# ushariRanasinghe/G2VLM

Hardware: AMD Instinct MI355X
Metric: views/sec (multi-view recon, G2VLM-2B-MoT) (higher is better)
Workload: dtype bf16; 1 GPU; C3: 8-view 518x518 reconstruction, full depth (24 DINO + 28 MoT + 15 decoder blocks), 1 scene per GPU; Lq=10968, Lk=10976, parallelism=replicas x1

## Files before the change

### g2vlm_amd/csrc/attn.hip

```cpp
#include <type_traits>
#include <utility>
#include "common.h"
#include "lds_dma.h"
#include "g2vlm_hip.h"

namespace {

#ifdef EXP_NO_EXP
#define G2V_EXP2(x) (x)
#else
#define G2V_EXP2(x) __builtin_amdgcn_exp2f(x)
#endif

constexpr int KV_TILE = 64;
constexpr int ROWB = 256;
constexpr int TILE_B = KV_TILE * ROWB;

struct FlashArgs {
  const __bf16* q; const __bf16* k; const __bf16* v; __bf16* o;
  const g2v_attn_tile* tiles;
  const g2v_attn_seg* segs;
  const int* seg_ptr;
  const int* comb;
  float* ws;
  int ldq, ldk, ldv, ldo, n_tiles, Hq, Hkv, n_blocks;
  float scale_log2;
#ifdef EXP_STAMPS
  unsigned long long* dbg;
  unsigned long long* clk;
  int dbg_pos;
#endif
};

#ifdef EXP_STAMPS
constexpr int STAMP_TILES = 24, STAMP_PTS = 8;
unsigned long long* g_attn_dbg = nullptr;
int g_attn_dbg_pos = -1;
unsigned long long* g_attn_clk = nullptr;
#define G2V_CLK_BEGIN() const unsigned long long clk_c0 = __builtin_amdgcn_s_memtime(), clk_r0 = __builtin_amdgcn_s_memrealtime()
#define G2V_CLK_END(lbv, wv) do { if (a.clk && (wv) == 0 && (threadIdx.x & 63) == 0) { a.clk[2 * (lbv)] = __builtin_amdgcn_s_memtime() - clk_c0; \
    a.clk[2 * (lbv) + 1] = __builtin_amdgcn_s_memrealtime() - clk_r0; } } while (0)
// ... 521 lines not shown
          const int kr = min(kt * KV_TILE + piece_row(i), T.k_len - 1);
          dma16_vaddr(base + ((size_t)kr * a.ldk + piece_col(i)) * 2, __builtin_amdgcn_readfirstlane(lds_addr(dst)) + piece_dst(i));
        }
      }
    };

    stage_any(kbase, smK, kt0);
    stage_any(vbase, smV, kt0);
    if (kt0 + 1 < kt1) { stage_any(kbase, smK, kt0 + 1); stage_any(vbase, smV, kt0 + 1); }
    if (kt0 + 2 < kt1) stage_any(kbase, smK, kt0 + 2);

    {
      auto q_to_acc = [&](auto qb_t) {
        constexpr int qb = decltype(qb_t)::value;
        const int qi = min(64 * wu + 32 * qb + r, T.q_rows - 1);
        const __bf16* qp = a.q + (size_t)(T.q0 + qi) * a.ldq + head * D + 8 * hh;
        u32x4 qv[KSTEPS];
#pragma unroll
        for (int ks = 0; ks < KSTEPS; ++ks) qv[ks] = *reinterpret_cast<const u32x4*>(qp + 16 * ks);
        auto put = [&](auto ks_t) {
          constexpr int ks = decltype(ks_t)::value, R = ACC_Q + 4 * (8 * qb + ks);
          acc_write<R>(qv[ks][0]); acc_write<R + 1>(qv[ks][1]); acc_write<R + 2>(qv[ks][2]); acc_write<R + 3>(qv[ks][3]);
        };
        put(std::integral_constant<int, 0>{}); put(std::integral_constant<int, 1>{}); put(std::integral_constant<int, 2>{});
        put(std::integral_constant<int, 3>{}); put(std::integral_constant<int, 4>{}); put(std::integral_constant<int, 5>{});
        put(std::integral_constant<int, 6>{}); put(std::integral_constant<int, 7>{});
      };
      q_to_acc(std::integral_constant<int, 0>{});
      q_to_acc(std::integral_constant<int, 1>{});
      acc_zero_seq<ACC_O>(std::make_integer_sequence<int, 128>{});
      acc_zero_seq<ACC_L>(std::make_integer_sequence<int, 32>{});
      wait32();
    }
    const int kmax0 = (T.q0 - T.q_win0) + 64 * wu + r + T.causal_shift;
// ... 332 lines not shown
          const float wgt = __builtin_amdgcn_exp2f(mv[u] - M);
          L = fmaf(lv[u], wgt, L);
#pragma unroll
          for (int e = 0; e < 4; ++e) acc[e] = fmaf(ov[u][e], wgt, acc[e]);
        }
      }
    }
    const float inv = 1.0f / L;
    __bf16* op = a.o + (size_t)(T.q0 + q) * a.ldo + head * D + 4 * c;
    *reinterpret_cast<u32x2*>(op) = u32x2{pack_bf16x2(acc[0] * inv, acc[1] * inv), pack_bf16x2(acc[2] * inv, acc[3] * inv)};
  }
}

int g_attn_form = 1;

template <int D>
int launch_flash(const FlashArgs& a, int n_comb, int waves, hipStream_t s) {
  if (a.n_blocks > 0) {
    if (D == 128 && waves == 8 && g_attn_form == 1 && a.ldk == a.ldv) hipLaunchKernelGGL(flash_fwd64_kernel, dim3(a.n_blocks), dim3(256), 0, s, a);
    else if (waves == 8) hipLaunchKernelGGL((flash_fwd_kernel<D, 8>), dim3(a.n_blocks), dim3(512), 0, s, a);
    else hipLaunchKernelGGL((flash_fwd_kernel<D, 4>), dim3(a.n_blocks), dim3(256), 0, s, a);
    G2V_CHECK_LAUNCH();
  }
  if (n_comb > 0) {
    hipLaunchKernelGGL(flash_combine_kernel<D>, dim3(n_comb, (32 * waves + COMB_ROWS - 1) / COMB_ROWS), dim3(256), 0, s, a);
    G2V_CHECK_LAUNCH();
  }
  return G2V_OK;
}

}

#ifdef EXP_STAMPS
extern "C" int g2v_debug_attn_stamps(void* buf) { g_attn_dbg = (unsigned long long*)buf; return 0; }
extern "C" int g2v_debug_attn_stamp_pos(int pos) { g_attn_dbg_pos = pos; return 0; }
extern "C" int g2v_debug_attn_clock(void* buf) { g_attn_clk = (unsigned long long*)buf; return 0; }
#endif

extern "C" int g2v_debug_attn_form(int form) { g_attn_form = form; return 0; }

extern "C" int64_t g2v_flash_attn_workspace(int n_slots) { return (int64_t)(n_slots > 0 ? n_slots : 0) * SLOT_FLOATS * 4; }

extern "C" int g2v_flash_attn(const void* q, int ldq, const void* k, int ldk, const void* v, int ldv, void* o, int ldo,
                              const g2v_attn_tile* tiles, int n_tiles, int Hq, int Hkv, int D, float scale,
                              const g2v_attn_seg* segs, const int32_t* seg_ptr, int n_blocks, const int32_t* comb, int n_comb,
                              int tile_rows, void* workspace, void* stream) {
  if (!q || !k || !v || !o || !tiles || n_tiles < 0 || Hq <= 0 || Hkv <= 0 || Hq % Hkv || n_blocks < 0 || n_comb < 0) return G2V_ERR_ARG;
  if ((n_blocks > 0 && (!segs || !seg_ptr)) || (n_comb > 0 && (!comb || !workspace))) return G2V_ERR_ARG;
  if ((ldq & 7) || (ldk & 7) || (ldv & 7) || (ldo & 3)) return G2V_ERR_ARG;
  if (tile_rows != 128 && tile_rows != 256) return G2V_ERR_ARG;
  if (n_tiles == 0 || (n_blocks == 0 && n_comb == 0)) return G2V_OK;
  FlashArgs a{(const __bf16*)q, (const __bf16*)k, (const __bf16*)v, (__bf16*)o, tiles, segs, seg_ptr, comb,
              (float*)workspace, ldq, ldk, ldv, ldo, n_tiles, Hq, Hkv, n_blocks, scale * 1.4426950408889634f};
#ifdef EXP_STAMPS
  a.dbg = g_attn_dbg;
  a.dbg_pos = g_attn_dbg_pos;
  a.clk = g_attn_clk;
#endif
  const int waves = tile_rows / 32;
  hipStream_t s = (hipStream_t)stream;
  switch (D) {
    case 16: return launch_flash<16>(a, n_comb, waves, s);
    case 64: return launch_flash<64>(a, n_comb, waves, s);
    case 80: return launch_flash<80>(a, n_comb, waves, s);
    case 96: return launch_flash<96>(a, n_comb, waves, s);
    case 128: return launch_flash<128>(a, n_comb, waves, s);
    default: return G2V_ERR_ARG;
  }
}
```

### g2vlm_amd/csrc/common.h

```cpp
#pragma once
#include <hip/hip_runtime.h>
#include <stdint.h>

typedef __attribute__((ext_vector_type(8))) __bf16 bf16x8;
typedef __attribute__((ext_vector_type(4))) __bf16 bf16x4;
typedef __attribute__((ext_vector_type(2))) __bf16 bf16x2;
typedef __attribute__((ext_vector_type(4))) short s16x4;
typedef __attribute__((ext_vector_type(4))) float f32x4;
typedef __attribute__((ext_vector_type(16))) float f32x16;
typedef __attribute__((ext_vector_type(4))) uint32_t u32x4;
typedef __attribute__((ext_vector_type(2))) uint32_t u32x2;

#define G2V_OK 0
#define G2V_ERR_ARG (-22)
#define G2V_ERR_LAUNCH (-5)

#define G2V_CHECK_LAUNCH()                         \
  do {                                             \
    hipError_t e__ = hipGetLastError();            \
    if (e__ != hipSuccess) return G2V_ERR_LAUNCH;  \
  } while (0)

__device__ __forceinline__ float bf2f(__bf16 x) { return (float)x; }
__device__ __forceinline__ __bf16 f2bf(float x) { return (__bf16)x; }
__device__ __forceinline__ float bfround(float x) {
  uint32_t r;
  asm("v_cvt_pk_bf16_f32 %0, %1, %1" : "=v"(r) : "v"(x));
  return __uint_as_float(r << 16);
}

__device__ __forceinline__ float bits2f_hi(uint32_t w) { return __uint_as_float(w & 0xffff0000u); }
__device__ __forceinline__ float bits2f_lo(uint32_t w) { return __uint_as_float(w << 16); }

__device__ __forceinline__ uint32_t pack_bf16x2(float lo, float hi) {
  bf16x2 v = {(__bf16)lo, (__bf16)hi};
  return *reinterpret_cast<uint32_t*>(&v);
}

__device__ __forceinline__ float wave_sum(float v) {
#pragma unroll
  for (int o = 32; o > 0; o >>= 1) v += __shfl_xor(v, o, 64);
  return v;
}
__device__ __forceinline__ float wave_max(float v) {
#pragma unroll
  for (int o = 32; o > 0; o >>= 1) v = fmaxf(v, __shfl_xor(v, o, 64));
  return v;
}

__device__ __forceinline__ float gelu_erf(float x) { return 0.5f * x * (1.0f + erff(x * 0.70710678118654752440f)); }
__device__ __forceinline__ float gelu_fast(float x) {
  const float a = fabsf(x) * 0.70710678118654752440f;
  const float t = __builtin_amdgcn_rcpf(fmaf(0.5f, a, 1.0f));
// ... 19 lines not shown
```

### g2vlm_amd/csrc/norm_rope.hip

```cpp
#include "common.h"
#include "g2vlm_hip.h"

namespace {


template <bool IN_BF16, int MAXV>
__device__ __forceinline__ int load_row(const void* x, size_t row_off, int C, int lane, f32x4 (&v)[MAXV]) {
  int n = 0;
#pragma unroll
  for (int i = 0; i < MAXV; ++i) {
    int c = (i * 64 + lane) * 4;
    v[i] = f32x4{0.f, 0.f, 0.f, 0.f};
    if (c < C) {
      if constexpr (IN_BF16) {
        u32x2 w = *reinterpret_cast<const u32x2*>(reinterpret_cast<const __bf16*>(x) + row_off + c);
        v[i] = f32x4{bits2f_lo(w[0]), bits2f_hi(w[0]), bits2f_lo(w[1]), bits2f_hi(w[1])};
      } else {
        v[i] = *reinterpret_cast<const f32x4*>(reinterpret_cast<const float*>(x) + row_off + c);
      }
      n = i + 1;
    }
  }
  return n;
}
// ... 89 lines not shown
  const int nh = Hq + 2 * Hkv;
  const long item = ((long)blockIdx.x * 256 + threadIdx.x) >> 4;
  const bool live = item < (long)L * nh;
  const long it = live ? item : 0;
  const int row = (int)(it / nh), h = (int)(it - (long)row * nh);
  const int j = threadIdx.x & 15;
  const __bf16* src = qkv + (size_t)row * nh * 128 + h * 128 + 4 * j;
  u32x2 a = *reinterpret_cast<const u32x2*>(src), b = *reinterpret_cast<const u32x2*>(src + 64);
  if (h >= Hq + Hkv) {
    if (live) {
      __bf16* dst = v_cache + ((size_t)kv_rows[row] * Hkv + (h - Hq - Hkv)) * 128 + 4 * j;
      *reinterpret_cast<u32x2*>(dst) = a; *reinterpret_cast<u32x2*>(dst + 64) = b;
    }
    return;
  }
  float x0[4] = {bits2f_lo(a[0]), bits2f_hi(a[0]), bits2f_lo(a[1]), bits2f_hi(a[1])};
  float x1[4] = {bits2f_lo(b[0]), bits2f_hi(b[0]), bits2f_lo(b[1]), bits2f_hi(b[1])};
  float ss = 0.f;
#pragma unroll
  for (int e = 0; e < 4; ++e) ss += x0[e] * x0[e] + x1[e] * x1[e];
#pragma unroll
  for (int o = 8; o > 0; o >>= 1) ss += __shfl_xor(ss, o, 64);
  const float rstd = 1.0f / sqrtf(ss / 128.f + eps);
  const bool isq = h < Hq;
  const float* w = (isq ? (row < split ? qw_lo : qw_hi) : (row < split ? kw_lo : kw_hi)) + 4 * j;
  const f32x4 w0 = *reinterpret_cast<const f32x4*>(w), w1 = *reinterpret_cast<const f32x4*>(w + 64);
  const float* cp = cs + (size_t)row * 128 + 4 * j; const float* sp = sn + (size_t)row * 128 + 4 * j;
  const f32x4 c0 = *reinterpret_cast<const f32x4*>(cp), c1 = *reinterpret_cast<const f32x4*>(cp + 64);
  const f32x4 s0 = *reinterpret_cast<const f32x4*>(sp), s1 = *reinterpret_cast<const f32x4*>(sp + 64);
  float o0[4], o1[4];
#pragma unroll
  for (int e = 0; e < 4; ++e) {
    float n0 = __fmul_rn(x0[e], rstd), n1 = __fmul_rn(x1[e], rstd);
    if (und_rounding) { n0 = bfround(n0); n1 = bfround(n1); }
    n0 = __fmul_rn(w0[e], n0); n1 = __fmul_rn(w1[e], n1);
    o0[e] = __fadd_rn(__fmul_rn(n0, c0[e]), __fmul_rn(-n1, s0[e]));
    o1[e] = __fadd_rn(__fmul_rn(n1, c1[e]), __fmul_rn(n0, s1[e]));
  }
  if (live) {
    __bf16* dst = (isq ? q_out + ((size_t)row * Hq + h) * 128 : k_cache + ((size_t)kv_rows[row] * Hkv + (h - Hq)) * 128) + 4 * j;
    *reinterpret_cast<u32x2*>(dst) = u32x2{pack_bf16x2(o0[0], o0[1]), pack_bf16x2(o0[2], o0[3])};
    *reinterpret_cast<u32x2*>(dst + 64) = u32x2{pack_bf16x2(o1[0], o1[1]), pack_bf16x2(o1[2], o1[3])};
  }
}

__global__ void rope2d_kernel(__bf16* x, int ld, int M, int col0, int n_heads, int D, const __bf16* cs, const __bf16* sn,
                              const int* pos, int P) {
  const int half = D / 2, quarter = D / 4;
  int per_row = n_heads * half;
  long i = (long)blockIdx.x * blockDim.x + threadIdx.x;
  if (i >= (long)M * per_row) return;
  int row = (int)(i / per_row), r = (int)(i - (long)row * per_row);
  int h = r / half, e = r - h * half;
  int axis = e / quarter, j = e - axis * quarter;
  int p = pos[(row % P) * 2 + axis];
  __bf16* t = x + (size_t)row * ld + col0 + h * D + axis * half;
  float t0 = bf2f(t[j]), t1 = bf2f(t[j + quarter]);
// ... 97 lines not shown
                                      const void* kw_lo, const void* kw_hi, int split, float eps, int und_rounding,
                                      const void* cos, const void* sin, void* q_out, void* k_cache, void* v_cache,
                                      const void* kv_rows, void* stream) {
  if (!qkv || !qw_lo || !qw_hi || !kw_lo || !kw_hi || !cos || !sin || !q_out || !k_cache || !v_cache || !kv_rows ||
      L < 0 || Hq <= 0 || Hkv <= 0) return G2V_ERR_ARG;
  if (L == 0) return G2V_OK;
  long items = (long)L * (Hq + 2 * Hkv);
  hipLaunchKernelGGL(qknorm_mrope_cache_kernel, dim3((unsigned)((items + 15) / 16)), dim3(256), 0, (hipStream_t)stream,
                     (const __bf16*)qkv, L, Hq, Hkv, (const float*)qw_lo, (const float*)qw_hi, (const float*)kw_lo,
                     (const float*)kw_hi, split, eps, und_rounding, (const float*)cos, (const float*)sin, (__bf16*)q_out,
                     (__bf16*)k_cache, (__bf16*)v_cache, (const int*)kv_rows);
  G2V_CHECK_LAUNCH();
  return G2V_OK;
}

extern "C" int g2v_rope2d(void* x, int ld, int M, int col0, int n_heads, int D, const void* cos, const void* sin,
                          const void* pos, int P, void* stream) {
  if (!x || !cos || !sin || !pos || M < 0 || n_heads <= 0 || D <= 0 || (D & 3) || P <= 0) return G2V_ERR_ARG;
  if (M == 0) return G2V_OK;
  long n = (long)M * n_heads * (D / 2);
  if ((D & 15) == 0 && (ld & 3) == 0 && (col0 & 3) == 0 && (reinterpret_cast<uintptr_t>(x) & 7) == 0 &&
      ((reinterpret_cast<uintptr_t>(cos) | reinterpret_cast<uintptr_t>(sin)) & 7) == 0) {
    n /= 4;
    hipLaunchKernelGGL(rope2d_vec4_kernel, dim3((unsigned)((n + 255) / 256)), dim3(256), 0, (hipStream_t)stream, (__bf16*)x, ld, M,
                       col0, n_heads, D, (const __bf16*)cos, (const __bf16*)sin, (const int*)pos, P);
    G2V_CHECK_LAUNCH();
    return G2V_OK;
  }
  hipLaunchKernelGGL(rope2d_kernel, dim3((unsigned)((n + 255) / 256)), dim3(256), 0, (hipStream_t)stream, (__bf16*)x, ld, M, col0,
                     n_heads, D, (const __bf16*)cos, (const __bf16*)sin, (const int*)pos, P);
// ... 14 lines not shown
```

### g2vlm_amd/engine.py

```python
import math
import os

import torch

from . import hip
from .decode import Decode, KVCache, linear_names, weight_key


def rope2d_tables(D, seq_len, base=100.0):
    inv_freq = 1.0 / (base ** (torch.arange(0, D, 2).float() / D))
    t = torch.arange(seq_len, dtype=inv_freq.dtype)
    freqs = torch.einsum("i,j->ij", t, inv_freq).to(torch.bfloat16)
    freqs = torch.cat((freqs, freqs), dim=-1)
    return freqs.cos(), freqs.sin()


def attn_tile_rows(windows, Hq):
    long_kv = sum(w[3] for w in windows if w[0] == windows[0][0]) >= 2048 and max(w[1] for w in windows) >= 2048
    tall = False
    if not long_kv:
        pad = lambda t: sum((w[1] + t - 1) // t * t for w in windows) / max(1, sum(w[1] for w in windows))
        items = sum((w[1] + 255) // 256 for w in windows) * Hq
        tall = items >= 512 and pad(256) <= 1.12 * pad(128)
    return 256 if (long_kv or tall) else 128
# ... 119 lines not shown
            assert not causal and local_kv is not None
            r0, nr = local_kv
            wins = [(0, L, r0, nr, False, 0)]
            if r0 > 0:
                wins.append((0, L, 0, r0, False, 1))
            if r0 + nr < tot:
                wins.append((0, L, r0 + nr, tot - r0 - nr, False, 1))
            plan = self.plan(tuple(wins), Hq)
        elif windows is not None:
            plan = self.plan(tuple(windows), Hq)
        else:
            plan = self.plan(((0, L, 0, tot, bool(causal)),), Hq)
        nq, nqkv = Hq * 128, (Hq + 2 * Hkv) * 128
        h = torch.empty((L, H), dtype=torch.bfloat16, device=self.dev)
        qkv = torch.empty((L, nqkv), dtype=torch.bfloat16, device=self.dev)
        qb = torch.empty((L, nq), dtype=torch.bfloat16, device=self.dev)
        ao = torch.empty((L, nq), dtype=torch.bfloat16, device=self.dev)
        act = torch.empty((L, Lc["ffn"]), dtype=torch.bfloat16, device=self.dev)
        ng, nu = split, L - split

        def groups(A, C, wname, bname=None, res=None, gamma=None, lda=None, ldc=None):
            gs = []
            for tag, r0, m, gam in (("geo", 0, ng, gamma), ("und", split, nu, None)):
                if m == 0:
                    continue
                gs.append(dict(A=A[r0:], W=w[wname.format(tag)], bias=w[bname.format(tag)] if bname else None,
                               C=C[r0:], res=res[r0:] if res is not None else None, gamma=gam, M=m))
            return gs

        for i in range(Lc["layers"] if num_layers is None else num_layers):
            p = f"L{i}."
            hp.rmsnorm(x, w[p + "geo.ln1"], w[p + "und.ln1"], split, eps, out=h)
            hp.gemm_bf16(groups(h, qkv, p + "{}.qkv.w", p + "{}.qkv.b"), nqkv, H, hp.EPI_BF16, out_ld=nqkv)
            hp.qknorm_mrope_cache(qkv, Hq, Hkv, w[p + "geo.qn"], w[p + "und.qn"], w[p + "geo.kn"], w[p + "und.kn"], split, eps,
                                  und_rounding, cos, sin, qb, cache.k[i], cache.v[i], kv_rows)
            if self.attn_events is not None:
                ev = (torch.cuda.Event(enable_timing=True), torch.cuda.Event(enable_timing=True))
                ev[0].record()
            kk, vv_ = cache.k[i][:tot].view(tot, Hkv * 128), cache.v[i][:tot].view(tot, Hkv * 128)
            if kv_exchange is not None:
                kv_exchange.start(i)
                hp.flash_attn(qb, kk, vv_, ao, plan, Hq, Hkv, 128, phase=0)
                kv_exchange.wait(i)
                for ph in range(1, len(plan.phases)):
                    hp.flash_attn(qb, kk, vv_, ao, plan, Hq, Hkv, 128, phase=ph)
            else:
                hp.flash_attn(qb, kk, vv_, ao, plan, Hq, Hkv, 128)
            if self.attn_events is not None:
                ev[1].record()
                self.attn_events.append((ev, L, tot))
            hp.gemm_bf16(groups(ao, x, p + "{}.o.w", None, res=x, gamma=w[p + "ls1"]), H, nq, hp.EPI_RES_F32, out_ld=H, ldres=H,
                         flags=hp.GAMMA_ROUND_BF16)
            hp.rmsnorm(x, w[p + "geo.ln2"], w[p + "und.ln2"], split, eps, out=h)
            if self.gemm_events is not None:
                gev = (torch.cuda.Event(enable_timing=True), torch.cuda.Event(enable_timing=True))
                gev[0].record()
            hp.gemm_bf16(groups(h, act, p + "{}.gu.w"), 2 * Lc["ffn"], H, hp.EPI_SWIGLU, out_ld=Lc["ffn"])
            if self.gemm_events is not None:
                gev[1].record()
                self.gemm_events.append((gev, L))
            hp.gemm_bf16(groups(act, x, p + "{}.down.w", None, res=x, gamma=w[p + "ls2"]), H, Lc["ffn"], hp.EPI_RES_F32, out_ld=H,
                         ldres=H, lda=Lc["ffn"], flags=hp.GAMMA_ROUND_BF16)
# ... 189 lines not shown
```

### g2vlm_amd/hip.py

```python
import ctypes as C
import os
import threading

import torch

_HERE = os.path.dirname(os.path.abspath(__file__))
LIB_PATH = os.environ.get("G2V_LIB_PATH") or os.path.join(_HERE, "lib", "libg2vlm_hip.so")

EPI_BF16, EPI_GELU, EPI_QUICKGELU, EPI_SWIGLU, EPI_RES_F32, EPI_RES_BF16 = range(6)
GAMMA_ROUND_BF16 = 1
FORCE_SMALL_TILE = 2
SUPERTILE = 4
FORCE_BIG_TILE = 8
FORCE_8P = 16
P8_H192, P8_H128, P8_H256, P8_TWO_BARRIER, P8_H288, P8_H224, P8_H160 = 128, 256, 512, 1024, 4096, 8192, 16384
P8_PIPELINED = 32768
P8_FOUR_WAVES = 65536
P8_EIGHT_WAVES = 131072
P8_NO_ROW_SKIP = 262144
F32, BF16 = 0, 1
NO_CAUSAL = 2 ** 30
_DEBUG_GEMM_FLAGS = int(os.environ.get("G2V_GEMM_FLAGS", "0"))


# ... 8 lines not shown
                ("flags", C.c_int32), ("workspace", C.c_void_p), ("workspace_bytes", C.c_int64)]


_P, _I, _F, _L = C.c_void_p, C.c_int, C.c_float, C.c_int64
_SIGS = {
    "g2v_version": ([], C.c_int),
    "g2v_arch": ([], C.c_char_p),
    "g2v_gemm_bf16": ([C.POINTER(GemmDesc), _P], C.c_int),
    "g2v_gemm_route": ([C.POINTER(GemmDesc), C.POINTER(C.c_int32 * 4)], C.c_int),
    "g2v_gemm_f32": ([_P, _P, _P, _P, _P, _I, _I, _I, _I, _I, _I, _I, _P], C.c_int),
    "g2v_layernorm": ([_P, _I, _I, _P, _P, _F, _P, _I, _I, _I, _I, _P], C.c_int),
    "g2v_rmsnorm": ([_P, _I, _P, _P, _I, _F, _P, _I, _I, _I, _I, _P], C.c_int),
    "g2v_mrope_table": ([_P, _I, _P, _P, _P, _P], C.c_int),
    "g2v_qknorm_mrope_cache": ([_P, _I, _I, _I, _P, _P, _P, _P, _I, _F, _I, _P, _P, _P, _P, _P, _P, _P], C.c_int),
    "g2v_flash_attn": ([_P, _I, _P, _I, _P, _I, _P, _I, _P, _I, _I, _I, _I, _F, _P, _P, _I, _P, _I, _I, _P, _P], C.c_int),
    "g2v_flash_attn_workspace": ([_I], C.c_int64),
    "g2v_debug_attn_form": ([_I], C.c_int),
    "g2v_rope2d": ([_P, _I, _I, _I, _I, _I, _P, _P, _P, _I, _P], C.c_int),
    "g2v_rope_vision": ([_P, _I, _I, _I, _I, _P, _P, _P], C.c_int),
    "g2v_im2col14": ([_P, _I, _I, _I, _P, _I, _P], C.c_int),
    "g2v_dino_preprocess": ([_P, _I, _I, _I, _I, C.POINTER(C.c_float), C.POINTER(C.c_float), _P, _P, _P], C.c_int),
    "g2v_dino_assemble": ([_P, _P, _P, _P, _P, _I, _I, _I, _P], C.c_int),
    "g2v_im2col_patch": ([_P, _I, _I, _I, _I, _P, _I, _P], C.c_int),
    "g2v_qwen_patchify_u8": ([_P, _I, _I, _I, C.POINTER(C.c_float), C.POINTER(C.c_float), _P, _I, _P], C.c_int),
    "g2v_vit_assemble": ([_P, _P, _P, _P, _I, _I, _I, _I, _P], C.c_int),
    "g2v_gather_rows_f32": ([_P, _I, _P, _P, _I, _I, _I, _P], C.c_int),
    "g2v_scatter_rows_f32": ([_P, _I, _P, _P, _I, _I, _I, _P], C.c_int),
    "g2v_cast_f32_bf16": ([_P, _P, _L, _P], C.c_int),
    "g2v_cast_bf16_f32": ([_P, _P, _L, _P], C.c_int),
    "g2v_pts_epilogue": ([_P, _I, _I, _I, _I, _P, _P, _P, _P], C.c_int),
# ... 194 lines not shown

def mrope_table(pos_i32, inv_freq):
    L = pos_i32.shape[1]
    cos = torch.empty((L, 128), dtype=torch.float32, device=pos_i32.device)
    sin = torch.empty_like(cos)
    _ck(lib().g2v_mrope_table(_p(pos_i32), L, _p(inv_freq), _p(cos), _p(sin), _stream()), "g2v_mrope_table")
    return cos, sin


def qknorm_mrope_cache(qkv, Hq, Hkv, qw_lo, qw_hi, kw_lo, kw_hi, split, eps, und_rounding, cos, sin, q_out, k_cache,
                       v_cache, kv_rows):
    L = qkv.shape[0]
    _ck(lib().g2v_qknorm_mrope_cache(_p(qkv), L, Hq, Hkv, _p(qw_lo), _p(qw_hi), _p(kw_lo), _p(kw_hi), int(split), eps,
                                     int(und_rounding), _p(cos), _p(sin), _p(q_out), _p(k_cache), _p(v_cache),
                                     _p(kv_rows), _stream()), "g2v_qknorm_mrope_cache")


class AttnSeg(C.Structure):
    _fields_ = [("desc", C.c_int32), ("head", C.c_int32), ("kt0", C.c_int32), ("kt1", C.c_int32), ("slot", C.c_int32),
                ("_pad", C.c_int32 * 3)]


class AttnPlan:

    def __init__(self, tiles, n_tiles, phases, comb, n_comb, n_slots, tile_rows, device):
        self.tiles, self.n_tiles, self.phases = tiles, n_tiles, phases
        self.comb, self.n_comb, self.n_slots, self.tile_rows = comb, n_comb, n_slots, tile_rows
        self.n_blocks = max((p[2] for p in phases), default=0)
        self.n_split = n_comb
        self.ws_words = max(4, int(lib().g2v_flash_attn_workspace(n_slots)) // 4)
# ... 103 lines not shown
        ptr, k = [0], 0
        for lst in per_block:
            for (i, kt0, kt1) in lst:
                d, h = items[i][0], items[i][1]
                sg = segs[k]
                sg.desc, sg.head, sg.kt0, sg.kt1, sg.slot = d, h, kt0, kt1, slot_of[(d, h, kt0)]
                k += 1
            ptr.append(k)
        seg_t = torch.frombuffer(bytearray(bytes(segs)), dtype=torch.int32).clone()
        phases.append((h2d(seg_t, device, resident=True), h2d(torch.tensor(ptr, dtype=torch.int32), device, resident=True), n_blocks))
    tiles = h2d(torch.tensor(rows, dtype=torch.int32).reshape(-1, 8), device, resident=True)
    comb_t = h2d(torch.tensor(comb if comb else [0, 0, 0, 0], dtype=torch.int32), device, resident=True)
    return AttnPlan(tiles, n_tiles, phases, comb_t, len(comb) // 4, n_slots, tile_rows, device)


def flash_attn(q, k, v, out, plan, Hq, Hkv, D, scale=None, phase=None):
    scale = scale if scale is not None else D ** -0.5
    ws = plan.ws(scratch_owner(q.device.index))
    last = len(plan.phases) - 1
    for i in (range(len(plan.phases)) if phase is None else (phase,)):
        segs, seg_ptr, n_blocks = plan.phases[i]
        n_comb = plan.n_comb if i == last else 0
        _ck(lib().g2v_flash_attn(_p(q), _rowmajor(q), _p(k), _rowmajor(k), _p(v), _rowmajor(v), _p(out), _rowmajor(out),
                                 _p(plan.tiles), plan.n_tiles, Hq, Hkv, D, scale, _p(segs), _p(seg_ptr), n_blocks, _p(plan.comb), n_comb,
                                 plan.tile_rows, _p(ws), _stream()), "g2v_flash_attn")
    return out


def rope2d(x, col0, n_heads, D, cos, sin, pos, P):
    _ck(lib().g2v_rope2d(_p(x), _rowmajor(x), x.shape[0], col0, n_heads, D, _p(cos), _p(sin), _p(pos), P, _stream()),
        "g2v_rope2d")


def rope_vision(x, n_heads, D, cos, sin):
    _ck(lib().g2v_rope_vision(_p(x), _rowmajor(x), x.shape[0], n_heads, D, _p(cos), _p(sin), _stream()), "g2v_rope_vision")


# ... 333 lines not shown
```

### include/g2vlm_hip.h

```cpp
#ifndef G2VLM_HIP_H
#define G2VLM_HIP_H
#include <stdint.h>
#ifdef __cplusplus
extern "C" {
#endif

int g2v_version(void);
const char* g2v_arch(void);

enum {
  G2V_EPI_BF16 = 0,
  G2V_EPI_GELU = 1,
  G2V_EPI_QUICKGELU = 2,
  G2V_EPI_SWIGLU = 3,
  G2V_EPI_RES_F32 = 4,
  G2V_EPI_RES_BF16 = 5
};
#define G2V_GEMM_GAMMA_ROUND_BF16 1
#define G2V_GEMM_SUPERTILE 4
#define G2V_GEMM_FORCE_BIG_TILE 8
#define G2V_GEMM_FORCE_8P 16
#define G2V_GEMM_8P_H192 128
#define G2V_GEMM_8P_H128 256
#define G2V_GEMM_8P_H256 512
// ... 32 lines not shown
                 int M, int N, int K, int lda, int ldc, int ldres, int relu, void* stream);

#define G2V_F32 0
#define G2V_BF16 1
int g2v_layernorm(const void* x, int x_dtype, int ldx, const void* w, const void* b, float eps,
                  void* out, int out_dtype, int ldo, int M, int C, void* stream);
int g2v_rmsnorm(const void* x, int ldx, const void* w_lo, const void* w_hi, int split, float eps,
                void* out, int out_dtype, int ldo, int M, int C, void* stream);

int g2v_mrope_table(const void* pos, int L, const void* inv_freq , void* cos, void* sin, void* stream);
int g2v_qknorm_mrope_cache(const void* qkv, int L, int Hq, int Hkv,
                           const void* qw_lo, const void* qw_hi, const void* kw_lo, const void* kw_hi,
                           int split, float eps, int und_rounding, const void* cos, const void* sin,
                           void* q_out, void* k_cache, void* v_cache, const void* kv_rows, void* stream);

typedef struct {
  int32_t q0, q_rows;
  int32_t k0, k_len;
  int32_t causal_shift;
  int32_t q_win0;
  int32_t _pad[2];
} g2v_attn_tile;

typedef struct {
  int32_t desc;
  int32_t head;
  int32_t kt0, kt1;
  int32_t slot;
  int32_t _pad[3];
} g2v_attn_seg;
int64_t g2v_flash_attn_workspace(int n_slots);
int g2v_debug_attn_form(int form);
int g2v_flash_attn(const void* q, int ldq, const void* k, int ldk, const void* v, int ldv,
                   void* o, int ldo, const g2v_attn_tile* tiles, int n_tiles,
                   int Hq, int Hkv, int D, float scale,
                   const g2v_attn_seg* segs, const int32_t* seg_ptr, int n_blocks, const int32_t* comb, int n_comb,
                   int tile_rows, void* workspace, void* stream);

int g2v_rope2d(void* x, int ld, int M, int col0, int n_heads, int D, const void* cos, const void* sin,
               const void* pos, int P, void* stream);

int g2v_rope_vision(void* x, int ld, int M, int n_heads, int D, const void* cos, const void* sin, void* stream);

int g2v_dino_preprocess(const void* in, int in_is_u8, int N, int H, int W, const float* mean3, const float* std3, void* norm,
                        void* orig, void* stream);

int g2v_lanczos_resize_u8(const void* src, int N, int Hin, int Win, void* dst, int Hout, int Wout, void* tmp,
                          const void* bounds_h, const void* kk_h, int ksize_h,
                          const void* bounds_v, const void* kk_v, int ksize_v, void* stream);
int g2v_im2col14(const void* img, int N, int H, int W, void* out, int Kpad, void* stream);
int g2v_dino_assemble(const void* patch, const void* cls, const void* regs, const void* pos,
                      void* x, int N, int P, int C, void* stream);

// ... 88 lines not shown
```

Before: 105.1 views/s.

## Fuse Q RMSNorm and mRoPE into flash attention Q load

Q-head RMSNorm and mRoPE move out of the separate qknorm_mrope_cache kernel and into the fwd64 attention kernel's Q-load prologue. Attention reads raw Q straight from the qkv buffer. A new K-only norm/rope kernel still fills the KV cache and copies V. This drops the round trip of the normalized Q buffer through memory and removes its allocation. In exchange every attention block recomputes the norm and rope for its Q rows, repeated per KV segment or phase, which adds register pressure to the hot kernel. The rounding also changes from explicit _rn ops to fmaf.

```diff
diff --git a/g2vlm_amd/csrc/attn.hip b/g2vlm_amd/csrc/attn.hip
--- a/g2vlm_amd/csrc/attn.hip
+++ b/g2vlm_amd/csrc/attn.hip
@@ -25,6 +25,9 @@
   float* ws;
   int ldq, ldk, ldv, ldo, n_tiles, Hq, Hkv, n_blocks;
   float scale_log2;
+  const float* qw_lo; const float* qw_hi; const float* cs; const float* sn;
+  int split, und_rounding;
+  float eps;
 #ifdef EXP_STAMPS
   unsigned long long* dbg;
   unsigned long long* clk;
@@ -576,10 +579,41 @@
       auto q_to_acc = [&](auto qb_t) {
         constexpr int qb = decltype(qb_t)::value;
         const int qi = min(64 * wu + 32 * qb + r, T.q_rows - 1);
-        const __bf16* qp = a.q + (size_t)(T.q0 + qi) * a.ldq + head * D + 8 * hh;
+        const int qrow = T.q0 + qi;
+        const __bf16* qp = a.q + (size_t)qrow * a.ldq + head * D + 8 * hh;
         u32x4 qv[KSTEPS];
 #pragma unroll
         for (int ks = 0; ks < KSTEPS; ++ks) qv[ks] = *reinterpret_cast<const u32x4*>(qp + 16 * ks);
+        if (a.cs != nullptr) {
+          float wsum[2];
+#pragma unroll
+          for (int b = 0; b < 2; ++b) {
+            float sq[4];
+#pragma unroll
+            for (int ks = 0; ks < 4; ++ks)
+              sq[ks] = qk_quad_sumsq(u32x2{qv[ks][2 * b], qv[ks][2 * b + 1]}, u32x2{qv[ks + 4][2 * b], qv[ks + 4][2 * b + 1]});
+            const float v4 = (sq[0] + sq[2]) + (sq[1] + sq[3]);
+            auto sw = __builtin_amdgcn_permlane32_swap(__float_as_uint(v4), __float_as_uint(v4), false, false);
+            wsum[b] = __uint_as_float(sw[0]) + __uint_as_float(sw[1]);
+          }
+          const float rstd = qk_rstd128(wsum[0] + wsum[1], a.eps);
+          const float* wp = (qrow < a.split ? a.qw_lo : a.qw_hi) + 8 * hh;
+          const float* cp = a.cs + (size_t)qrow * 128 + 8 * hh;
+          const float* sp = a.sn + (size_t)qrow * 128 + 8 * hh;
+#pragma unroll
+          for (int ks = 0; ks < 4; ++ks) {
+#pragma unroll
+            for (int b = 0; b < 2; ++b) {
+              const int d = 16 * ks + 4 * b;
+              const f32x4 w0 = *reinterpret_cast<const f32x4*>(wp + d), w1 = *reinterpret_cast<const f32x4*>(wp + 64 + d);
+              const f32x4 cc = *reinterpret_cast<const f32x4*>(cp + d), ss = *reinterpret_cast<const f32x4*>(sp + d);
+              u32x2 xa = {qv[ks][2 * b], qv[ks][2 * b + 1]}, xb = {qv[ks + 4][2 * b], qv[ks + 4][2 * b + 1]};
+              qk_quad_norm_rope(xa, xb, rstd, a.und_rounding, w0, w1, cc, cc, ss, ss);
+              qv[ks][2 * b] = xa[0]; qv[ks][2 * b + 1] = xa[1];
+              qv[ks + 4][2 * b] = xb[0]; qv[ks + 4][2 * b + 1] = xb[1];
+            }
+          }
+        }
         auto put = [&](auto ks_t) {
           constexpr int ks = decltype(ks_t)::value, R = ACC_Q + 4 * (8 * qb + ks);
           acc_write<R>(qv[ks][0]); acc_write<R + 1>(qv[ks][1]); acc_write<R + 2>(qv[ks][2]); acc_write<R + 3>(qv[ks][3]);
@@ -942,10 +976,12 @@
 
 int g_attn_form = 1;
 
+bool takes_fwd64(int D, int waves, int ldk, int ldv) { return D == 128 && waves == 8 && g_attn_form == 1 && ldk == ldv; }
+
 template <int D>
 int launch_flash(const FlashArgs& a, int n_comb, int waves, hipStream_t s) {
   if (a.n_blocks > 0) {
-    if (D == 128 && waves == 8 && g_attn_form == 1 && a.ldk == a.ldv) hipLaunchKernelGGL(flash_fwd64_kernel, dim3(a.n_blocks), dim3(256), 0, s, a);
+    if (takes_fwd64(D, waves, a.ldk, a.ldv)) hipLaunchKernelGGL(flash_fwd64_kernel, dim3(a.n_blocks), dim3(256), 0, s, a);
     else if (waves == 8) hipLaunchKernelGGL((flash_fwd_kernel<D, 8>), dim3(a.n_blocks), dim3(512), 0, s, a);
     else hipLaunchKernelGGL((flash_fwd_kernel<D, 4>), dim3(a.n_blocks), dim3(256), 0, s, a);
     G2V_CHECK_LAUNCH();
@@ -969,17 +1005,24 @@
 
 extern "C" int64_t g2v_flash_attn_workspace(int n_slots) { return (int64_t)(n_slots > 0 ? n_slots : 0) * SLOT_FLOATS * 4; }
 
-extern "C" int g2v_flash_attn(const void* q, int ldq, const void* k, int ldk, const void* v, int ldv, void* o, int ldo,
-                              const g2v_attn_tile* tiles, int n_tiles, int Hq, int Hkv, int D, float scale,
-                              const g2v_attn_seg* segs, const int32_t* seg_ptr, int n_blocks, const int32_t* comb, int n_comb,
-                              int tile_rows, void* workspace, void* stream) {
+namespace {
+int flash_attn_impl(const void* q, int ldq, const void* k, int ldk, const void* v, int ldv, void* o, int ldo,
+                    const g2v_attn_tile* tiles, int n_tiles, int Hq, int Hkv, int D, float scale, const g2v_attn_seg* segs,
+                    const int32_t* seg_ptr, int n_blocks, const int32_t* comb, int n_comb, int tile_rows, void* workspace,
+                    const g2v_attn_qprep* qp, void* stream) {
   if (!q || !k || !v || !o || !tiles || n_tiles < 0 || Hq <= 0 || Hkv <= 0 || Hq % Hkv || n_blocks < 0 || n_comb < 0) return G2V_ERR_ARG;
   if ((n_blocks > 0 && (!segs || !seg_ptr)) || (n_comb > 0 && (!comb || !workspace))) return G2V_ERR_ARG;
   if ((ldq & 7) || (ldk & 7) || (ldv & 7) || (ldo & 3)) return G2V_ERR_ARG;
   if (tile_rows != 128 && tile_rows != 256) return G2V_ERR_ARG;
+  if (qp && (!qp->qw_lo || !qp->qw_hi || !qp->cos || !qp->sin || !takes_fwd64(D, tile_rows / 32, ldk, ldv))) return G2V_ERR_ARG;
   if (n_tiles == 0 || (n_blocks == 0 && n_comb == 0)) return G2V_OK;
   FlashArgs a{(const __bf16*)q, (const __bf16*)k, (const __bf16*)v, (__bf16*)o, tiles, segs, seg_ptr, comb,
-              (float*)workspace, ldq, ldk, ldv, ldo, n_tiles, Hq, Hkv, n_blocks, scale * 1.4426950408889634f};
+              (float*)workspace, ldq, ldk, ldv, ldo, n_tiles, Hq, Hkv, n_blocks, scale * 1.4426950408889634f,
+              nullptr, nullptr, nullptr, nullptr, 0, 0, 0.f};
+  if (qp) {
+    a.qw_lo = (const float*)qp->qw_lo; a.qw_hi = (const float*)qp->qw_hi; a.cs = (const float*)qp->cos; a.sn = (const float*)qp->sin;
+    a.split = qp->split; a.und_rounding = qp->und_rounding; a.eps = qp->eps;
+  }
 #ifdef EXP_STAMPS
   a.dbg = g_attn_dbg;
   a.dbg_pos = g_attn_dbg_pos;
@@ -996,3 +1039,25 @@
     default: return G2V_ERR_ARG;
   }
 }
+}
+
+extern "C" int g2v_flash_attn(const void* q, int ldq, const void* k, int ldk, const void* v, int ldv, void* o, int ldo,
+                              const g2v_attn_tile* tiles, int n_tiles, int Hq, int Hkv, int D, float scale,
+                              const g2v_attn_seg* segs, const int32_t* seg_ptr, int n_blocks, const int32_t* comb, int n_comb,
+                              int tile_rows, void* workspace, void* stream) {
+  return flash_attn_impl(q, ldq, k, ldk, v, ldv, o, ldo, tiles, n_tiles, Hq, Hkv, D, scale, segs, seg_ptr, n_blocks, comb, n_comb,
+                         tile_rows, workspace, nullptr, stream);
+}
+
+extern "C" int g2v_flash_attn_qprep_supported(int D, int tile_rows, int ldk, int ldv) {
+  return (tile_rows == 128 || tile_rows == 256) && takes_fwd64(D, tile_rows / 32, ldk, ldv) ? 1 : 0;
+}
+
+extern "C" int g2v_flash_attn_qprep(const void* qkv, int ldq, const void* k, int ldk, const void* v, int ldv, void* o, int ldo,
+                                    const g2v_attn_tile* tiles, int n_tiles, int Hq, int Hkv, int D, float scale,
+                                    const g2v_attn_seg* segs, const int32_t* seg_ptr, int n_blocks, const int32_t* comb,
+                                    int n_comb, int tile_rows, void* workspace, const g2v_attn_qprep* qprep, void* stream) {
+  if (!qprep) return G2V_ERR_ARG;
+  return flash_attn_impl(qkv, ldq, k, ldk, v, ldv, o, ldo, tiles, n_tiles, Hq, Hkv, D, scale, segs, seg_ptr, n_blocks, comb, n_comb,
+                         tile_rows, workspace, qprep, stream);
+}
diff --git a/g2vlm_amd/csrc/common.h b/g2vlm_amd/csrc/common.h
--- a/g2vlm_amd/csrc/common.h
+++ b/g2vlm_amd/csrc/common.h
@@ -37,6 +37,31 @@
   return *reinterpret_cast<uint32_t*>(&v);
 }
 
+__device__ __forceinline__ float qk_quad_sumsq(u32x2 a, u32x2 b) {
+  const float t0 = fmaf(bits2f_lo(a[0]), bits2f_lo(a[0]), bits2f_lo(b[0]) * bits2f_lo(b[0]));
+  const float t1 = fmaf(bits2f_hi(a[0]), bits2f_hi(a[0]), bits2f_hi(b[0]) * bits2f_hi(b[0]));
+  const float t2 = fmaf(bits2f_lo(a[1]), bits2f_lo(a[1]), bits2f_lo(b[1]) * bits2f_lo(b[1]));
+  const float t3 = fmaf(bits2f_hi(a[1]), bits2f_hi(a[1]), bits2f_hi(b[1]) * bits2f_hi(b[1]));
+  return ((t0 + t1) + t2) + t3;
+}
+__device__ __forceinline__ float qk_rstd128(float ss, float eps) { return 1.0f / sqrtf(fmaf(ss, 0.0078125f, eps)); }
+__device__ __forceinline__ void qk_quad_norm_rope(u32x2& a, u32x2& b, float rstd, int und_rounding, f32x4 w0, f32x4 w1,
+                                                  f32x4 c0, f32x4 c1, f32x4 s0, f32x4 s1) {
+  const float x0[4] = {bits2f_lo(a[0]), bits2f_hi(a[0]), bits2f_lo(a[1]), bits2f_hi(a[1])};
+  const float x1[4] = {bits2f_lo(b[0]), bits2f_hi(b[0]), bits2f_lo(b[1]), bits2f_hi(b[1])};
+  float o0[4], o1[4];
+#pragma unroll
+  for (int e = 0; e < 4; ++e) {
+    float n0 = x0[e] * rstd, n1 = x1[e] * rstd;
+    if (und_rounding) { n0 = bfround(n0); n1 = bfround(n1); }
+    n0 = w0[e] * n0; n1 = w1[e] * n1;
+    o0[e] = fmaf(n0, c0[e], -(n1 * s0[e]));
+    o1[e] = fmaf(n0, s1[e], n1 * c1[e]);
+  }
+  a = u32x2{pack_bf16x2(o0[0], o0[1]), pack_bf16x2(o0[2], o0[3])};
+  b = u32x2{pack_bf16x2(o1[0], o1[1]), pack_bf16x2(o1[2], o1[3])};
+}
+
 __device__ __forceinline__ float wave_sum(float v) {
 #pragma unroll
   for (int o = 32; o > 0; o >>= 1) v += __shfl_xor(v, o, 64);
diff --git a/g2vlm_amd/csrc/norm_rope.hip b/g2vlm_amd/csrc/norm_rope.hip
--- a/g2vlm_amd/csrc/norm_rope.hip
+++ b/g2vlm_amd/csrc/norm_rope.hip
@@ -127,33 +127,56 @@
     }
     return;
   }
-  float x0[4] = {bits2f_lo(a[0]), bits2f_hi(a[0]), bits2f_lo(a[1]), bits2f_hi(a[1])};
-  float x1[4] = {bits2f_lo(b[0]), bits2f_hi(b[0]), bits2f_lo(b[1]), bits2f_hi(b[1])};
-  float ss = 0.f;
-#pragma unroll
-  for (int e = 0; e < 4; ++e) ss += x0[e] * x0[e] + x1[e] * x1[e];
+  float ss = qk_quad_sumsq(a, b);
 #pragma unroll
   for (int o = 8; o > 0; o >>= 1) ss += __shfl_xor(ss, o, 64);
-  const float rstd = 1.0f / sqrtf(ss / 128.f + eps);
+  const float rstd = qk_rstd128(ss, eps);
   const bool isq = h < Hq;
   const float* w = (isq ? (row < split ? qw_lo : qw_hi) : (row < split ? kw_lo : kw_hi)) + 4 * j;
   const f32x4 w0 = *reinterpret_cast<const f32x4*>(w), w1 = *reinterpret_cast<const f32x4*>(w + 64);
   const float* cp = cs + (size_t)row * 128 + 4 * j; const float* sp = sn + (size_t)row * 128 + 4 * j;
   const f32x4 c0 = *reinterpret_cast<const f32x4*>(cp), c1 = *reinterpret_cast<const f32x4*>(cp + 64);
   const f32x4 s0 = *reinterpret_cast<const f32x4*>(sp), s1 = *reinterpret_cast<const f32x4*>(sp + 64);
-  float o0[4], o1[4];
-#pragma unroll
-  for (int e = 0; e < 4; ++e) {
-    float n0 = __fmul_rn(x0[e], rstd), n1 = __fmul_rn(x1[e], rstd);
-    if (und_rounding) { n0 = bfround(n0); n1 = bfround(n1); }
-    n0 = __fmul_rn(w0[e], n0); n1 = __fmul_rn(w1[e], n1);
-    o0[e] = __fadd_rn(__fmul_rn(n0, c0[e]), __fmul_rn(-n1, s0[e]));
-    o1[e] = __fadd_rn(__fmul_rn(n1, c1[e]), __fmul_rn(n0, s1[e]));
-  }
+  qk_quad_norm_rope(a, b, rstd, und_rounding, w0, w1, c0, c1, s0, s1);
   if (live) {
     __bf16* dst = (isq ? q_out + ((size_t)row * Hq + h) * 128 : k_cache + ((size_t)kv_rows[row] * Hkv + (h - Hq)) * 128) + 4 * j;
-    *reinterpret_cast<u32x2*>(dst) = u32x2{pack_bf16x2(o0[0], o0[1]), pack_bf16x2(o0[2], o0[3])};
-    *reinterpret_cast<u32x2*>(dst + 64) = u32x2{pack_bf16x2(o1[0], o1[1]), pack_bf16x2(o1[2], o1[3])};
+    *reinterpret_cast<u32x2*>(dst) = a;
+    *reinterpret_cast<u32x2*>(dst + 64) = b;
+  }
+}
+
+__global__ __launch_bounds__(256) void knorm_mrope_cache_kernel(
+    const __bf16* qkv, int L, int Hq, int Hkv, const float* kw_lo, const float* kw_hi, int split, float eps, int und_rounding,
+    const float* cs, const float* sn, __bf16* k_cache, __bf16* v_cache, const int* kv_rows) {
+  const int nh = 2 * Hkv;
+  const long item = ((long)blockIdx.x * 256 + threadIdx.x) >> 4;
+  const bool live = item < (long)L * nh;
+  const long it = live ? item : 0;
+  const int row = (int)(it / nh), h = (int)(it - (long)row * nh);
+  const int j = threadIdx.x & 15;
+  const __bf16* src = qkv + ((size_t)row * (Hq + nh) + Hq + h) * 128 + 4 * j;
+  u32x2 a = *reinterpret_cast<const u32x2*>(src), b = *reinterpret_cast<const u32x2*>(src + 64);
+  if (h >= Hkv) {
+    if (live) {
+      __bf16* dst = v_cache + ((size_t)kv_rows[row] * Hkv + (h - Hkv)) * 128 + 4 * j;
+      *reinterpret_cast<u32x2*>(dst) = a; *reinterpret_cast<u32x2*>(dst + 64) = b;
+    }
+    return;
+  }
+  float ss = qk_quad_sumsq(a, b);
+#pragma unroll
+  for (int o = 8; o > 0; o >>= 1) ss += __shfl_xor(ss, o, 64);
+  const float rstd = qk_rstd128(ss, eps);
+  const float* w = (row < split ? kw_lo : kw_hi) + 4 * j;
+  const f32x4 w0 = *reinterpret_cast<const f32x4*>(w), w1 = *reinterpret_cast<const f32x4*>(w + 64);
+  const float* cp = cs + (size_t)row * 128 + 4 * j; const float* sp = sn + (size_t)row * 128 + 4 * j;
+  const f32x4 c0 = *reinterpret_cast<const f32x4*>(cp), c1 = *reinterpret_cast<const f32x4*>(cp + 64);
+  const f32x4 s0 = *reinterpret_cast<const f32x4*>(sp), s1 = *reinterpret_cast<const f32x4*>(sp + 64);
+  qk_quad_norm_rope(a, b, rstd, und_rounding, w0, w1, c0, c1, s0, s1);
+  if (live) {
+    __bf16* dst = k_cache + ((size_t)kv_rows[row] * Hkv + h) * 128 + 4 * j;
+    *reinterpret_cast<u32x2*>(dst) = a;
+    *reinterpret_cast<u32x2*>(dst + 64) = b;
   }
 }
 
@@ -281,6 +304,19 @@
   return G2V_OK;
 }
 
+extern "C" int g2v_knorm_mrope_cache(const void* qkv, int L, int Hq, int Hkv, const void* kw_lo, const void* kw_hi, int split,
+                                     float eps, int und_rounding, const void* cos, const void* sin, void* k_cache,
+                                     void* v_cache, const void* kv_rows, void* stream) {
+  if (!qkv || !kw_lo || !kw_hi || !cos || !sin || !k_cache || !v_cache || !kv_rows || L < 0 || Hq <= 0 || Hkv <= 0) return G2V_ERR_ARG;
+  if (L == 0) return G2V_OK;
+  long items = (long)L * 2 * Hkv;
+  hipLaunchKernelGGL(knorm_mrope_cache_kernel, dim3((unsigned)((items + 15) / 16)), dim3(256), 0, (hipStream_t)stream,
+                     (const __bf16*)qkv, L, Hq, Hkv, (const float*)kw_lo, (const float*)kw_hi, split, eps, und_rounding,
+                     (const float*)cos, (const float*)sin, (__bf16*)k_cache, (__bf16*)v_cache, (const int*)kv_rows);
+  G2V_CHECK_LAUNCH();
+  return G2V_OK;
+}
+
 extern "C" int g2v_rope2d(void* x, int ld, int M, int col0, int n_heads, int D, const void* cos, const void* sin,
                           const void* pos, int P, void* stream) {
   if (!x || !cos || !sin || !pos || M < 0 || n_heads <= 0 || D <= 0 || (D & 3) || P <= 0) return G2V_ERR_ARG;
diff --git a/g2vlm_amd/engine.py b/g2vlm_amd/engine.py
--- a/g2vlm_amd/engine.py
+++ b/g2vlm_amd/engine.py
@@ -5,6 +5,8 @@
 
 from . import hip
 from .decode import Decode, KVCache, linear_names, weight_key
+
+_ATTN_QPREP = os.environ.get("G2V_ATTN_QPREP", "1") != "0"
 
 
 def rope2d_tables(D, seq_len, base=100.0):
@@ -157,7 +159,8 @@
         nq, nqkv = Hq * 128, (Hq + 2 * Hkv) * 128
         h = torch.empty((L, H), dtype=torch.bfloat16, device=self.dev)
         qkv = torch.empty((L, nqkv), dtype=torch.bfloat16, device=self.dev)
-        qb = torch.empty((L, nq), dtype=torch.bfloat16, device=self.dev)
+        qprep = _ATTN_QPREP and hp.flash_attn_qprep_supported(plan, 128, Hkv * 128, Hkv * 128)
+        qb = None if qprep else torch.empty((L, nq), dtype=torch.bfloat16, device=self.dev)
         ao = torch.empty((L, nq), dtype=torch.bfloat16, device=self.dev)
         act = torch.empty((L, Lc["ffn"]), dtype=torch.bfloat16, device=self.dev)
         ng, nu = split, L - split
@@ -175,20 +178,26 @@
             p = f"L{i}."
             hp.rmsnorm(x, w[p + "geo.ln1"], w[p + "und.ln1"], split, eps, out=h)
             hp.gemm_bf16(groups(h, qkv, p + "{}.qkv.w", p + "{}.qkv.b"), nqkv, H, hp.EPI_BF16, out_ld=nqkv)
-            hp.qknorm_mrope_cache(qkv, Hq, Hkv, w[p + "geo.qn"], w[p + "und.qn"], w[p + "geo.kn"], w[p + "und.kn"], split, eps,
-                                  und_rounding, cos, sin, qb, cache.k[i], cache.v[i], kv_rows)
+            if qprep:
+                hp.knorm_mrope_cache(qkv, Hq, Hkv, w[p + "geo.kn"], w[p + "und.kn"], split, eps, und_rounding, cos, sin,
+                                     cache.k[i], cache.v[i], kv_rows)
+                qin, qp = qkv, (w[p + "geo.qn"], w[p + "und.qn"], split, eps, und_rounding, cos, sin)
+            else:
+                hp.qknorm_mrope_cache(qkv, Hq, Hkv, w[p + "geo.qn"], w[p + "und.qn"], w[p + "geo.kn"], w[p + "und.kn"], split, eps,
+                                      und_rounding, cos, sin, qb, cache.k[i], cache.v[i], kv_rows)
+                qin, qp = qb, None
             if self.attn_events is not None:
                 ev = (torch.cuda.Event(enable_timing=True), torch.cuda.Event(enable_timing=True))
                 ev[0].record()
             kk, vv_ = cache.k[i][:tot].view(tot, Hkv * 128), cache.v[i][:tot].view(tot, Hkv * 128)
             if kv_exchange is not None:
                 kv_exchange.start(i)
-                hp.flash_attn(qb, kk, vv_, ao, plan, Hq, Hkv, 128, phase=0)
+                hp.flash_attn(qin, kk, vv_, ao, plan, Hq, Hkv, 128, phase=0, qprep=qp)
                 kv_exchange.wait(i)
                 for ph in range(1, len(plan.phases)):
-                    hp.flash_attn(qb, kk, vv_, ao, plan, Hq, Hkv, 128, phase=ph)
+                    hp.flash_attn(qin, kk, vv_, ao, plan, Hq, Hkv, 128, phase=ph, qprep=qp)
             else:
-                hp.flash_attn(qb, kk, vv_, ao, plan, Hq, Hkv, 128)
+                hp.flash_attn(qin, kk, vv_, ao, plan, Hq, Hkv, 128, qprep=qp)
             if self.attn_events is not None:
                 ev[1].record()
                 self.attn_events.append((ev, L, tot))
diff --git a/g2vlm_amd/hip.py b/g2vlm_amd/hip.py
--- a/g2vlm_amd/hip.py
+++ b/g2vlm_amd/hip.py
@@ -46,6 +46,9 @@
     "g2v_mrope_table": ([_P, _I, _P, _P, _P, _P], C.c_int),
     "g2v_qknorm_mrope_cache": ([_P, _I, _I, _I, _P, _P, _P, _P, _I, _F, _I, _P, _P, _P, _P, _P, _P, _P], C.c_int),
     "g2v_flash_attn": ([_P, _I, _P, _I, _P, _I, _P, _I, _P, _I, _I, _I, _I, _F, _P, _P, _I, _P, _I, _I, _P, _P], C.c_int),
+    "g2v_knorm_mrope_cache": ([_P, _I, _I, _I, _P, _P, _I, _F, _I, _P, _P, _P, _P, _P, _P], C.c_int),
+    "g2v_flash_attn_qprep": ([_P, _I, _P, _I, _P, _I, _P, _I, _P, _I, _I, _I, _I, _F, _P, _P, _I, _P, _I, _I, _P, _P, _P], C.c_int),
+    "g2v_flash_attn_qprep_supported": ([_I, _I, _I, _I], C.c_int),
     "g2v_flash_attn_workspace": ([_I], C.c_int64),
     "g2v_debug_attn_form": ([_I], C.c_int),
     "g2v_rope2d": ([_P, _I, _I, _I, _I, _I, _P, _P, _P, _I, _P], C.c_int),
@@ -270,6 +273,17 @@
     _ck(lib().g2v_qknorm_mrope_cache(_p(qkv), L, Hq, Hkv, _p(qw_lo), _p(qw_hi), _p(kw_lo), _p(kw_hi), int(split), eps,
                                      int(und_rounding), _p(cos), _p(sin), _p(q_out), _p(k_cache), _p(v_cache),
                                      _p(kv_rows), _stream()), "g2v_qknorm_mrope_cache")
+
+
+def knorm_mrope_cache(qkv, Hq, Hkv, kw_lo, kw_hi, split, eps, und_rounding, cos, sin, k_cache, v_cache, kv_rows):
+    L = qkv.shape[0]
+    _ck(lib().g2v_knorm_mrope_cache(_p(qkv), L, Hq, Hkv, _p(kw_lo), _p(kw_hi), int(split), eps, int(und_rounding), _p(cos),
+                                    _p(sin), _p(k_cache), _p(v_cache), _p(kv_rows), _stream()), "g2v_knorm_mrope_cache")
+
+
+class AttnQPrep(C.Structure):
+    _fields_ = [("qw_lo", C.c_void_p), ("qw_hi", C.c_void_p), ("cos", C.c_void_p), ("sin", C.c_void_p),
+                ("split", C.c_int32), ("und_rounding", C.c_int32), ("eps", C.c_float), ("_pad", C.c_int32)]
 
 
 class AttnSeg(C.Structure):
@@ -403,13 +417,27 @@
     return AttnPlan(tiles, n_tiles, phases, comb_t, len(comb) // 4, n_slots, tile_rows, device)
 
 
-def flash_attn(q, k, v, out, plan, Hq, Hkv, D, scale=None, phase=None):
+def flash_attn_qprep_supported(plan, D, ldk, ldv):
+    return bool(lib().g2v_flash_attn_qprep_supported(D, plan.tile_rows, ldk, ldv))
+
+
+def flash_attn(q, k, v, out, plan, Hq, Hkv, D, scale=None, phase=None, qprep=None):
     scale = scale if scale is not None else D ** -0.5
+    if qprep is not None:
+        qw_lo, qw_hi, split, eps, und_rounding, cos, sin = qprep
+        assert cos.shape[0] >= q.shape[0] and cos.shape[1] == 128 and cos.is_contiguous() and sin.is_contiguous()
+        qp = AttnQPrep(qw_lo.data_ptr(), qw_hi.data_ptr(), cos.data_ptr(), sin.data_ptr(), int(split), int(und_rounding), eps, 0)
     ws = plan.ws(scratch_owner(q.device.index))
     last = len(plan.phases) - 1
     for i in (range(len(plan.phases)) if phase is None else (phase,)):
         segs, seg_ptr, n_blocks = plan.phases[i]
         n_comb = plan.n_comb if i == last else 0
+        if qprep is not None:
+            _ck(lib().g2v_flash_attn_qprep(_p(q), _rowmajor(q), _p(k), _rowmajor(k), _p(v), _rowmajor(v), _p(out), _rowmajor(out),
+                                           _p(plan.tiles), plan.n_tiles, Hq, Hkv, D, scale, _p(segs), _p(seg_ptr), n_blocks,
+                                           _p(plan.comb), n_comb, plan.tile_rows, _p(ws), C.byref(qp), _stream()),
+                "g2v_flash_attn_qprep")
+            continue
         _ck(lib().g2v_flash_attn(_p(q), _rowmajor(q), _p(k), _rowmajor(k), _p(v), _rowmajor(v), _p(out), _rowmajor(out),
                                  _p(plan.tiles), plan.n_tiles, Hq, Hkv, D, scale, _p(segs), _p(seg_ptr), n_blocks, _p(plan.comb), n_comb,
                                  plan.tile_rows, _p(ws), _stream()), "g2v_flash_attn")
diff --git a/include/g2vlm_hip.h b/include/g2vlm_hip.h
--- a/include/g2vlm_hip.h
+++ b/include/g2vlm_hip.h
@@ -70,6 +70,10 @@
                            int split, float eps, int und_rounding, const void* cos, const void* sin,
                            void* q_out, void* k_cache, void* v_cache, const void* kv_rows, void* stream);
 
+int g2v_knorm_mrope_cache(const void* qkv, int L, int Hq, int Hkv, const void* kw_lo, const void* kw_hi,
+                          int split, float eps, int und_rounding, const void* cos, const void* sin,
+                          void* k_cache, void* v_cache, const void* kv_rows, void* stream);
+
 typedef struct {
   int32_t q0, q_rows;
   int32_t k0, k_len;
@@ -93,6 +97,20 @@
                    const g2v_attn_seg* segs, const int32_t* seg_ptr, int n_blocks, const int32_t* comb, int n_comb,
                    int tile_rows, void* workspace, void* stream);
 
+typedef struct {
+  const void* qw_lo; const void* qw_hi;
+  const void* cos; const void* sin;
+  int32_t split, und_rounding;
+  float eps;
+  int32_t _pad;
+} g2v_attn_qprep;
+int g2v_flash_attn_qprep_supported(int D, int tile_rows, int ldk, int ldv);
+int g2v_flash_attn_qprep(const void* qkv, int ldq, const void* k, int ldk, const void* v, int ldv,
+                         void* o, int ldo, const g2v_attn_tile* tiles, int n_tiles,
+                         int Hq, int Hkv, int D, float scale,
+                         const g2v_attn_seg* segs, const int32_t* seg_ptr, int n_blocks, const int32_t* comb, int n_comb,
+                         int tile_rows, void* workspace, const g2v_attn_qprep* qprep, void* stream);
+
 int g2v_rope2d(void* x, int ld, int M, int col0, int n_heads, int D, const void* cos, const void* sin,
                const void* pos, int P, void* stream);
 
```

Result: no change. 105.0 views/s (-0.1%).
